# flynn-nrg/izpi

Measured on AMD Instinct MI355X. Metric: Msamples/sec (pixels x spp) at 1024x1024/512spp, higher is better.
Workload: dtype f64

## Files before the change

### include/izpi_gpu.h

```cpp
#ifndef IZPI_GPU_H
#define IZPI_GPU_H
#include <stddef.h>
#include <stdint.h>
#include "izpi_types.h"

#ifdef __cplusplus
extern "C" {
#endif

typedef struct izpi_ctx izpi_ctx;

typedef struct izpi_scene_desc {
  uint32_t abi_version;
  uint32_t num_nodes;
  uint32_t num_prims;
  uint32_t num_tris, num_spheres, num_lights, num_materials, num_textures;
  uint32_t num_spd;
  uint32_t flags;
  uint64_t num_texels;
  const izpi_bvh4_node* nodes;
  const uint32_t* prim_ref;
  const double* tri_v0;
  const double* tri_v1;
  const double* tri_v2;
// ... 29 lines not shown
  IZPI_SAMPLER_WIREFRAME = 3,
  IZPI_SAMPLER_ALBEDO = 4,
  IZPI_SAMPLER_SPECTRAL = 5
};
enum {
  IZPI_OUT_CANVAS = 0,
  IZPI_OUT_PACKED = 1
};

typedef struct izpi_render_tuning {
  uint32_t slots;
  uint32_t chunk_units;
  uint32_t rec_dense;
  uint32_t pool_div;
  uint32_t trace_chunk;
  uint32_t refill_min;
  uint32_t prim_weight;
  uint32_t flags;
  uint64_t tail_paths;
  uint32_t peer_timeout_ms;
  uint32_t pad_tuning;
} izpi_render_tuning;
enum {
  IZPI_TUNE_NO_DIST = 1,
  IZPI_TUNE_GENERAL_TRACE = 2,
  IZPI_TUNE_NO_LEAF_SHORTCUT = 4,
  IZPI_TUNE_SCALAR_SLAB = 8,
  IZPI_TUNE_NO_TAIL = 16,
  IZPI_TUNE_PASS_LOG = 32,
  IZPI_TUNE_NO_LDS_BVH = 64,
  IZPI_TUNE_NO_RAY_LDS = 128,
  IZPI_TUNE_NO_PRIM_LDS = 256,
  IZPI_TUNE_NO_PLACE_PICK = 512,
  IZPI_TUNE_NO_QNODES = 1024
};

typedef struct izpi_render_req {
  uint32_t width, height;
  uint32_t spp;
  uint32_t max_depth;
  uint32_t sampler;
  uint32_t out_layout;
  uint32_t num_tiles;
  uint32_t num_bg_spd;
  const uint32_t* tiles;
  const double* bg_spd_wavelengths;
  const double* bg_spd_values;
  double background[3];
  uint64_t seed;
  uint32_t post;
  uint32_t abi_version;
  double exposure;
  const izpi_render_tuning* tuning;
  uint32_t accumulation;
  uint32_t pad_req;
  double ink[3];
} izpi_render_req;

enum { IZPI_ACC_RECURSIVE = 0, IZPI_ACC_FORWARD = 1 };

enum { IZPI_POST_NONE = 0, IZPI_POST_SPECTRAL = 1,
       IZPI_POST_GAMMA_CLAMP = 2 };

enum { IZPI_FILTER_GAMMA = 1,
       IZPI_FILTER_CLAMP = 2   };
#define IZPI_MAX_FILTERS 8

// ... 85 lines not shown
```

### izpi_amd/_native.py

```python
import ctypes as C
from pathlib import Path

ROOT = Path(__file__).resolve().parents[1]
LIB_PATH = ROOT / "izpi_amd" / "_lib" / "libizpi_gpu.so"

c_double_p = C.POINTER(C.c_double)
c_uint32_p = C.POINTER(C.c_uint32)
c_float_p = C.POINTER(C.c_float)

COMM_ID_BYTES = 128
IZPI_OK, IZPI_ERR_INVALID, IZPI_ERR_HIP, IZPI_ERR_NO_SCENE, IZPI_ERR_UNSUPPORTED, IZPI_ERR_DEVICE, IZPI_ERR_PEER = range(7)
IZPI_ABI_VERSION = 4
ACC_RECURSIVE, ACC_FORWARD = 0, 1
SCENE_QUANTIZED_BVH = 1
PRIM_TRIANGLE, PRIM_SPHERE = 0, 1
TEX_CONSTANT, TEX_IMAGE, TEX_SPECTRAL_GAUSSIAN, TEX_SPECTRAL_TABULATED, TEX_SPECTRAL_IMAGE = 1, 3, 5, 7, 9
MAT_DIELECTRIC, MAT_DIFFUSE_LIGHT, MAT_ISOTROPIC, MAT_LAMBERT, MAT_METAL, MAT_PBR = 1, 2, 3, 4, 5, 6
MATF_BEER_LAMBERT = 1
SAMPLER_NORMAL, SAMPLER_COLOUR, SAMPLER_WIREFRAME, SAMPLER_ALBEDO, SAMPLER_SPECTRAL = 1, 2, 3, 4, 5
OUT_CANVAS, OUT_PACKED = 0, 1
POST_NONE, POST_SPECTRAL, POST_GAMMA_CLAMP = 0, 1, 2
FILTER_GAMMA, FILTER_CLAMP = 1, 2
MAX_FILTERS = 8
HOST_SKIP_BVH = 1
# ... 31 lines not shown
                ("vertical", C.c_double * 3), ("u", C.c_double * 3), ("v", C.c_double * 3),
                ("lens_radius", C.c_double), ("time0", C.c_double), ("time1", C.c_double), ("exposure", C.c_double)]


class SceneDesc(C.Structure):
    _fields_ = [("abi_version", C.c_uint32), ("num_nodes", C.c_uint32), ("num_prims", C.c_uint32),
                ("num_tris", C.c_uint32), ("num_spheres", C.c_uint32), ("num_lights", C.c_uint32),
                ("num_materials", C.c_uint32), ("num_textures", C.c_uint32), ("num_spd", C.c_uint32),
                ("flags", C.c_uint32), ("num_texels", C.c_uint64),
                ("nodes", C.POINTER(BVH4Node)), ("prim_ref", c_uint32_p),
                ("tri_v0", c_double_p), ("tri_v1", c_double_p), ("tri_v2", c_double_p),
                ("tri_e1", c_double_p), ("tri_e2", c_double_p), ("tri_normal", c_double_p),
                ("tri_tangent", c_double_p), ("tri_bitangent", c_double_p), ("tri_uv", c_double_p),
                ("tri_area", c_double_p), ("tri_mat", c_uint32_p),
                ("sph_center0", c_double_p), ("sph_center1", c_double_p), ("sph_time", c_double_p),
                ("sph_radius", c_double_p), ("sph_mat", c_uint32_p),
                ("light_ref", c_uint32_p), ("materials", C.POINTER(Material)), ("textures", C.POINTER(Texture)),
                ("texels", c_double_p), ("spd_wavelengths", c_double_p), ("spd_values", c_double_p),
                ("camera", Camera)]


class RenderTuning(C.Structure):
    _fields_ = [("slots", C.c_uint32), ("chunk_units", C.c_uint32), ("rec_dense", C.c_uint32),
                ("pool_div", C.c_uint32), ("trace_chunk", C.c_uint32), ("refill_min", C.c_uint32),
                ("prim_weight", C.c_uint32), ("flags", C.c_uint32), ("tail_paths", C.c_uint64),
                ("peer_timeout_ms", C.c_uint32), ("pad_tuning", C.c_uint32)]


TUNE_NO_DIST, TUNE_GENERAL_TRACE, TUNE_NO_LEAF_SHORTCUT, TUNE_SCALAR_SLAB, TUNE_NO_TAIL, TUNE_PASS_LOG = 1, 2, 4, 8, 16, 32
TUNE_NO_LDS_BVH = 64
TUNE_NO_RAY_LDS = 128
TUNE_NO_PRIM_LDS = 256
TUNE_NO_QNODES = 1024


def tuning(**kw):
    t = RenderTuning()
    for k, v in kw.items():
        if k == "flags" and not isinstance(v, int):
            v = sum(v)
        setattr(t, k, v)
    return t


class RenderReq(C.Structure):
    _fields_ = [("width", C.c_uint32), ("height", C.c_uint32), ("spp", C.c_uint32), ("max_depth", C.c_uint32),
                ("sampler", C.c_uint32), ("out_layout", C.c_uint32), ("num_tiles", C.c_uint32),
                ("num_bg_spd", C.c_uint32), ("tiles", c_uint32_p), ("bg_spd_wavelengths", c_double_p),
                ("bg_spd_values", c_double_p), ("background", C.c_double * 3), ("seed", C.c_uint64),
                ("post", C.c_uint32), ("abi_version", C.c_uint32), ("exposure", C.c_double),
                ("tuning", C.POINTER(RenderTuning)), ("accumulation", C.c_uint32), ("pad_req", C.c_uint32),
                ("ink", C.c_double * 3)]


class RenderStats(C.Structure):
    _fields_ = [("rays", C.c_uint64), ("node_visits", C.c_uint64), ("tri_tests", C.c_uint64),
                ("sph_tests", C.c_uint64), ("light_tri_tests", C.c_uint64), ("light_sph_tests", C.c_uint64),
                ("samples", C.c_uint64), ("kernel_ms", C.c_double), ("shade_ms", C.c_double),
                ("total_ms", C.c_double), ("launches", C.c_uint32), ("pad", C.c_uint32),
                ("node_steps", C.c_uint64), ("prim_steps", C.c_uint64), ("leaf_shortcuts", C.c_uint64),
                ("tail_ms", C.c_double), ("tail_node_visits", C.c_uint64), ("tail_tri_tests", C.c_uint64),
                ("tail_sph_tests", C.c_uint64), ("parks", C.c_uint64), ("workspace_bytes", C.c_uint64),
                ("scene_bytes", C.c_uint64), ("slots", C.c_uint32), ("rec_dense", C.c_uint32),
                ("pool_blocks", C.c_uint32), ("chunk_spp", C.c_uint32), ("alloc_ms", C.c_double)]

    def as_dict(self):
# ... 200 lines not shown
```

### izpi_amd/csrc/izpi_gpu.hip

```cpp
#include "izpi_kern.h"

__global__ void __launch_bounds__(256) k_spectral_post(const double* in, double* out, uint32_t W, uint32_t H,
                                                       double exposure) {
  __shared__ double ys[18][18];
  const int tx = threadIdx.x & 15, ty = threadIdx.x >> 4;
  const int x0 = blockIdx.x * 16, y0 = blockIdx.y * 16;
  for (int i = threadIdx.x; i < 18 * 18; i += 256) {
    const int hx = x0 + (i % 18) - 1, hy = y0 + (i / 18) - 1;
    ys[i / 18][i % 18] = (hx >= 0 && hx < (int)W && hy >= 0 && hy < (int)H) ? in[((size_t)hy * W + hx) * 4 + 1] : 0.0;
  }
  __syncthreads();
  const int x = x0 + tx, y = y0 + ty;
  if (x >= (int)W || y >= (int)H) return;
  const size_t pi = ((size_t)y * W + x) * 4;
  const double2 xy = *reinterpret_cast<const double2*>(in + pi), za = *reinterpret_cast<const double2*>(in + pi + 2);
  double X = xy.x, Y = xy.y, Z = za.x;
  const double cur = ys[ty + 1][tx + 1];
  if (cur > 0) {
    double nb[8];
    int nn = 0;
    for (int dy = -1; dy <= 1; dy++)
      for (int dx = -1; dx <= 1; dx++) {
        if (dx == 0 && dy == 0) continue;
        const int nx = x + dx, ny = y + dy;
// ... 634 lines not shown
    return IZPI_OK;
  }
  if (tu.flags & IZPI_TUNE_PASS_LOG) HIP_TRY(hipEventRecord(ctx->evb[0], ctx->stream));
  WaveBuf bufs[2];
  carve_state(ctx->d_state, slots, need_time, rec_pool != 0, need_cold, need_uv, thr_planes, bufs);
  hipStream_t st = ctx->stream;
  HIP_TRY(hipMemcpyAsync(ctx->d_tiles, tiles.data(), tiles.size() * sizeof(uint32_t), hipMemcpyHostToDevice, st));
  if (nbg) {
    HIP_TRY(hipMemcpyAsync(ctx->d_bg, req->bg_spd_wavelengths, nbg * sizeof(double), hipMemcpyHostToDevice, st));
    HIP_TRY(hipMemcpyAsync(ctx->d_bg + nbg, req->bg_spd_values, nbg * sizeof(double), hipMemcpyHostToDevice, st));
  }
  HIP_TRY(hipMemsetAsync(ctx->d_running, 0, (size_t)num_pixels * 3 * sizeof(double), st));
  HIP_TRY(hipMemsetAsync(ctx->d_counters, 0, CNT_N * sizeof(unsigned long long), st));
  HIP_TRY(hipMemsetAsync(ctx->d_cpart, 0, (size_t)cpart_rows * CNT_N * sizeof(unsigned long long), st));
  HIP_TRY(hipMemsetAsync(ctx->d_misc, 0, 8 * MISC_STRIDE * sizeof(uint32_t), st));

  ShadeParams sp{};
  sp.width = req->width; sp.height = req->height; sp.max_depth = req->max_depth;
  sp.tile_w = tw; sp.tile_h = th; sp.num_bg_spd = (uint32_t)nbg; sp.slots = slots;
  sp.bg_sorted = nbg >= 2;
  for (size_t i = 1; i < nbg; i++)
    if (!(req->bg_spd_wavelengths[i - 1] <= req->bg_spd_wavelengths[i])) sp.bg_sorted = 0;
  sp.tiles = ctx->d_tiles; sp.bg_wl = ctx->d_bg; sp.bg_val = ctx->d_bg + nbg;
  sp.background[0] = req->background[0]; sp.background[1] = req->background[1]; sp.background[2] = req->background[2];
  sp.rec_dense = rec_dense; sp.rec_pool = rec_pool;
  sp.pool_shift = 0;
  while (pool_blocks && (POOL_SHARDS << sp.pool_shift) < pool_blocks) sp.pool_shift++;
  sp.seed = req->seed; sp.out = ctx->d_samples; sp.recs = fwd ? nullptr : ctx->d_recs; sp.mat_const = sc.mat_const; sp.head = misc(ctx, 0);
  sp.num_mc = ctx->num_materials; sp.num_tex = ctx->num_textures; sp.num_spd = ctx->num_spd;
  sp.staged = ctx->num_materials <= MC_LDS && ctx->num_materials <= MAT_LDS && sc.num_lights <= LT_LDS &&
              ctx->num_textures <= TEX_LDS && ctx->num_spd <= SPD_LDS && nbg <= BG_LDS;
  sp.prims_staged = sc.num_prims <= PR_LDS && !(tuning_of(req).flags & IZPI_TUNE_NO_PRIM_LDS);
  if (sp.staged && (req->sampler == IZPI_SAMPLER_SPECTRAL || ctx->num_spd)) sp.staged = 2;
  sc.lds_bytes = sp.prims_staged ? lds_off::END : sp.staged == 2 ? lds_off::SPECTRAL_END : sp.staged ? lds_off::COLOUR_END : 0;
  sp.pool = rec_pool ? ctx->d_pool : nullptr; sp.pool_ring = rec_pool ? ctx->d_ring : nullptr;
  sp.pool_ctr = rec_pool ? ctx->d_pool_ctr : nullptr;
  sp.counters = ctx->d_counters; sp.cpart = ctx->d_cpart; sp.error = misc(ctx, 1);
  sp.finq = ctx->d_finq;
  WaveParams wp{};
  wp.in = bufs[0]; wp.out = bufs[1]; wp.trace_next = misc(ctx, 2); wp.slots = slots;
  wp.read_kind = !ctx->sc.no_pathlen ? 1u : 0u;
  wp.hit_uv = need_uv ? 1u : 0u;
  wp.pool_ctr = sp.pool_ctr;
  wp.cpart = ctx->d_cpart;
  AccumParams ap{};
  ap.num_pixels = num_pixels; ap.spp = req->spp; ap.width = req->width; ap.height = req->height;
  ap.tile_w = tw; ap.tile_h = th; ap.sampler = req->sampler; ap.out_layout = req->out_layout;
  ap.tiles = ctx->d_tiles; ap.samples = ctx->d_samples; ap.running = ctx->d_running; ap.out = out_dev;

  float trace_ms = 0, shade_ms = 0, tail_ms = 0;
  uint32_t launches = 0;
  const double t_launch = host_ms();
  HIP_TRY(hipEventRecord(ctx->ev0, st));
  if (tu.flags & IZPI_TUNE_PASS_LOG) {
    HIP_TRY(hipEventSynchronize(ctx->ev0));
    float prep = 0;
    HIP_TRY(hipEventElapsedTime(&prep, ctx->evb[0], ctx->ev0));
    fprintf(stderr, "IZPI_T ev0_synced %.3f prep_gpu_ms %.3f body_start %.3f\n", diag_clock_ms(), prep,
            diag_clock_ms() - host_ms());
  }
#define IZPI_RUN(S, F) run_sampler<S, F>(ctx, req, sc, tr, sp, wp, ap, num_pixels, chunk, pool_blocks, compact, &trace_ms, &shade_ms, \
                                        &tail_ms, &launches)
  if (req->sampler == IZPI_SAMPLER_COLOUR) rc = fwd ? IZPI_RUN(IZPI_SAMPLER_COLOUR, true) : IZPI_RUN(IZPI_SAMPLER_COLOUR, false);
  else rc = fwd ? IZPI_RUN(IZPI_SAMPLER_SPECTRAL, true) : IZPI_RUN(IZPI_SAMPLER_SPECTRAL, false);
#undef IZPI_RUN
  if (rc) return rc;
// ... 1139 lines not shown
```

### izpi_amd/csrc/izpi_kern.h

```cpp
#pragma once
#include <hip/hip_runtime.h>
#include <stdio.h>
#include <stdlib.h>
#include <string.h>
#include <algorithm>
#include <cmath>
#include <string>
#include <vector>

#include <rccl/rccl.h>

#include <atomic>
#include <chrono>
#include <thread>

#include "../../include/izpi_host.h"
#include "../../include/izpi_gpu_debug.h"
#include "izpi_dev.h"
#include "izpi_req.h"
#include "cie_tables.h"

using namespace izd;

#define HIP_TRY(expr)                                                                  \
// ... 55 lines not shown
#pragma unroll
    for (uint32_t i = 0; i < sizeof(T) / 8; i++) d[i] = q[i];
    return r;
  } else {
    return *(const __attribute__((address_space(3))) T*)p;
  }
}

template <bool L, class T>
IZPI_DEV T tld(const T* p) {
  if constexpr (L) return lds_ld(p);
  else return *p;
}
constexpr uint32_t MAT_LDS = 64, TEX_LDS = 64, SPD_LDS = 384, BG_LDS = 128, MT_LDS = 64, LT_LDS = 64, PR_LDS = 64;
namespace lds_off {
constexpr uint32_t al(uint64_t b) { return (uint32_t)((b + 31) & ~31ull); }
constexpr uint32_t MC = 0;
constexpr uint32_t MT = MC + al(MT_LDS * sizeof(double4));
constexpr uint32_t LT = MT + al(MT_LDS * sizeof(MatTex));
constexpr uint32_t LT2 = LT + al(LT_LDS * 16 * sizeof(double));
constexpr uint32_t MAT = LT2 + al(LT_LDS * 6 * sizeof(double));
constexpr uint32_t TEX = MAT + al(MAT_LDS * sizeof(izpi_material));
constexpr uint32_t COLOUR_END = TEX + al(TEX_LDS * sizeof(izpi_texture));
constexpr uint32_t SPD = COLOUR_END;
constexpr uint32_t SPDV = SPD + al(SPD_LDS * sizeof(double));
constexpr uint32_t CIE = SPDV + al(SPD_LDS * sizeof(double));
constexpr uint32_t BG = CIE + al(5 * IZPI_CIE_N * sizeof(double));
constexpr uint32_t BGV = BG + al(BG_LDS * sizeof(double));
constexpr uint32_t SPECTRAL_END = BGV + al(BG_LDS * sizeof(double));
constexpr uint32_t GS = SPECTRAL_END;
constexpr uint32_t TT = GS + al(PR_LDS * sizeof(GShade));
constexpr uint32_t GP = TT + al(PR_LDS * sizeof(GTriTex));
constexpr uint32_t END = GP + al(PR_LDS * sizeof(GPrim));
}
IZPI_DEV char* lds_arena() {
  extern __shared__ __attribute__((aligned(16))) char izpi_lds_arena[];
  return izpi_lds_arena;
}
IZPI_DEV izpi_material* mat_lds() { return (izpi_material*)(lds_arena() + lds_off::MAT); }
IZPI_DEV izpi_texture* tex_lds() { return (izpi_texture*)(lds_arena() + lds_off::TEX); }
IZPI_DEV double* spd_lds() { return (double*)(lds_arena() + lds_off::SPD); }
IZPI_DEV double* spdv_lds() { return (double*)(lds_arena() + lds_off::SPDV); }
IZPI_DEV double* cie_lds() { return (double*)(lds_arena() + lds_off::CIE); }
IZPI_DEV double* bg_lds() { return (double*)(lds_arena() + lds_off::BG); }
IZPI_DEV double* bgv_lds() { return (double*)(lds_arena() + lds_off::BGV); }
IZPI_DEV izpi_material mat_rec(const DevScene& sc, bool st, uint32_t m) {
  if (st) return lds_ld(mat_lds() + m);
  return sc.materials[m];
}
IZPI_DEV izpi_texture tex_rec(const DevScene& sc, bool st, int32_t id) {
  if (st) return lds_ld(tex_lds() + id);
  return sc.textures[id];
}

IZPI_DEV V3 image_rgb(const double* texels, uint64_t off, uint32_t w, uint32_t h, uint32_t fmt, double u, double v) {
  int64_t i = go_int(u * (double)w);
  int64_t j = go_int((1 - v) * ((double)h - 0.001));
  if (i < 0) i = 0;
  if (j < 0) j = 0;
  if (i > (int64_t)w - 1) i = (int64_t)w - 1;
  if (j > (int64_t)h - 1) j = (int64_t)h - 1;
  uint64_t k = (uint64_t)j * w + (uint64_t)i;
  if (fmt == TEXF_GRAY) {
    const double g = texels[off + k];
    return mk(g, g, g);
  }
// ... 1150 lines not shown
```

### izpi_amd/csrc/shade.h

```cpp
#pragma once
#include "izpi_kern.h"

template <int SAMPLER, bool FWD>
__global__ void __launch_bounds__(256) k_start(const DevScene sc, const ShadeParams sp_in, const WaveParams wp) {
  ShadeParams sp = sp_in;
  sp.staged = 0;
  sp.prims_staged = 0;
  const uint32_t j = blockIdx.x * 256 + threadIdx.x;
  bool want = j < sp.slots;
  bool push = false;
  bool first = true;
  PathSt P;
  RayRec R;
  P.rslot = j;
  for (;;) {
    uint32_t unit;
    if (first) {
      unit = (want && j < sp.total_units) ? j : 0xFFFFFFFFu;
      first = false;
    } else {
      unit = grab_unit(sp, want);
    }
    if (__ballot(want) == 0) break;
    if (want) {
// ... 68 lines not shown
  if (threadIdx.x == 0) {
    const uint32_t ne = np + nu;
    if (nu && u0 + nu >= sp.total_units) exhausted = true;
    s_pbase[b] = pb;
    s_ubase[b] = u0;
    s_granted[b] = u0 >= sp.total_units ? 0u : min(nu, sp.total_units - u0);
    s_nput[b] = np;
    s_nent[b] = ne;
    SCLK_VMWAIT();
    SCLK_ADD(SCLK_RATOM, rb1);
  }
  __syncthreads();
  SCLK_ADD(SCLK_RB2, rb1);
  uint32_t ur = (uint32_t)__popcll(mu & lt), pr = (uint32_t)__popcll(mp & lt);
  for (uint32_t i = 0; i < w; i++) { ur += s_u[b][i]; pr += s_p[b][i]; }
  if constexpr (QSEP) {
    q_rank = (uint32_t)__popcll(mq & lt);
    q_total = 0;
#pragma unroll
    for (uint32_t k = 0; k < SHADE_WAVES; k++) {
      q_rank += k < w ? s_q[b][k] : 0u;
      q_total += s_q[b][k];
    }
  } else {
    q_rank = ur;
    q_total = 0;
#pragma unroll
    for (uint32_t k = 0; k < SHADE_WAVES; k++) q_total += s_u[b][k];
  }
  const bool has_entry = unit_want && s_nput[b] + ur < s_nent[b];
  const bool granted = unit_want && ur < s_granted[b];
  unit = granted ? s_ubase[b] + ur : 0xFFFFFFFFu;
  pos = put ? s_pbase[b] + pr : (has_entry ? s_pbase[b] + s_nput[b] + ur : 0xFFFFFFFFu);
}

template <int SAMPLER, bool FWD>
IZPI_DEV void refill_one(const DevScene& sc, const ShadeParams& sp, const WaveBuf& out, uint32_t unit, uint32_t pos,
                         PathSt& P) {
  RayRec R;
  for (;;) {
    if (start_path<SAMPLER, FWD>(sc, sp, unit, P, R)) {
      store_entry<SAMPLER, FWD>(out, pos, P, R);
      return;
    }
    unit = atomicAdd(sp.head, 1u);
    if (unit >= sp.total_units) {
      dead_entry(out, pos);
      return;
    }
  }
}




template <int SAMPLER, int MATSET, bool DEFER, bool FWD>
IZPI_DEV void shade_item(const DevScene& sc, const ShadeParams& sp, const WaveBuf& in, uint32_t i, uint32_t kind,
                         const EntryIn& E, PathSt& P, RayRec& R, bool& push, bool& done, uint32_t& fblk, uint32_t& c_lt,
                         uint32_t& c_ls, bool& queued) {
  const bool COLOUR = SAMPLER == IZPI_SAMPLER_COLOUR;
  const bool st = sp.staged != 0;
  SCLK_T(sc0);
  SCLK_VMWAIT();
  SCLK_ADD(SCLK_ENTRY, sc0);
  for (int k = 0; k < 3; k++) { R.o[k] = E.ray.o[k]; R.d[k] = E.ray.d[k]; }
  R.kind = kind;
// ... 263 lines not shown
    const unsigned long long idx = atomicAdd(c, 1ull);
    if (idx < __atomic_load_n(c + 2, __ATOMIC_RELAXED)) return sp.pool_ring[((size_t)ring << sp.pool_shift) + (idx & size_mask)] + 1u;
  }
  return 0u;
}

template <int SAMPLER>
IZPI_DEV void fin_queue(unsigned long long* q, uint32_t j, const PathSt& P, const RayRec& R) {
  const bool colour = SAMPLER == IZPI_SAMPLER_COLOUR;
  q[j] = P.unit | (unsigned long long)P.rslot << 32;
  q[FINQ_CAP + j] = P.blk | (unsigned long long)(P.depth | P.zf << 16) << 32;
  q[2 * FINQ_CAP + j] = (unsigned long long)__double_as_longlong(R.o[0]);
  q[3 * FINQ_CAP + j] = (unsigned long long)__double_as_longlong(colour ? R.o[1] : P.lambda);
  q[4 * FINQ_CAP + j] = (unsigned long long)__double_as_longlong(colour ? R.o[2] : P.lpdf);
}
template <int SAMPLER, int MATSET>
IZPI_DEV void fin_flush(const ShadeParams& sp, const unsigned long long* q, uint32_t n) {
  const bool colour = SAMPLER == IZPI_SAMPLER_COLOUR;
  for (uint32_t j = threadIdx.x; j < n; j += SHADE_THREADS) {
    PathSt P;
    const unsigned long long w0 = q[j], w1 = q[FINQ_CAP + j];
    P.unit = (uint32_t)w0; P.rslot = (uint32_t)(w0 >> 32);
    P.blk = (uint32_t)w1; P.depth = (uint32_t)(w1 >> 32) & 0xFFFFu; P.zf = (uint32_t)(w1 >> 48);
    const double a = __longlong_as_double((long long)q[2 * FINQ_CAP + j]);
    const double b = __longlong_as_double((long long)q[3 * FINQ_CAP + j]);
    const double c = __longlong_as_double((long long)q[4 * FINQ_CAP + j]);
    P.lambda = colour ? 0.0 : b; P.lpdf = colour ? 0.0 : c;
    finish<SAMPLER, MATSET>(sp, P, colour ? mk(a, b, c) : mk(a, 0.0, 0.0));
    if (sp.rec_pool && P.blk) pool_free_one(sp, P.blk);
  }
}

constexpr int SHADE_WPE = 3;
template <int SAMPLER, int MATSET, bool FWD>
__global__ void __launch_bounds__(SHADE_THREADS) __attribute__((amdgpu_waves_per_eu(SHADE_WPE)))
k_shade(const DevScene sc, const ShadeParams sp, const WaveParams wp) {
  constexpr bool DREF = FWD;
  shade_stage(sc, sp);
  uint32_t parity = 0;
  const uint32_t n = *wp.in_count;
  const uint32_t cam_b = FWD && wp.cam ? wp.cam[0] : 0u, cam_u = FWD && wp.cam ? wp.cam[1] : 0u,
                 cam_m = FWD && wp.cam ? wp.cam[2] : 0u;
  if (blockIdx.x == 0 && threadIdx.x == 0) *wp.trace_next = 0;
  bool exhausted = false;
  uint32_t c_lt = 0, c_ls = 0, c_park = 0;
  const uint32_t stride = gridDim.x * SHADE_THREADS;
  constexpr bool DEFER = !FWD && (SAMPLER == IZPI_SAMPLER_SPECTRAL || ms_spec(MATSET));
  constexpr bool COLOUR_DEFER = DEFER && SAMPLER == IZPI_SAMPLER_COLOUR;
  unsigned long long* fq = sp.finq + (size_t)blockIdx.x * FINQ_WORDS * FINQ_CAP;
  uint32_t fq_n = 0;
#ifdef IZPI_SHADE_CLOCKS
  uint64_t k_item = 0, k_ref = 0, k_push = 0;
  sclk_zero();
#endif
  for (uint32_t base = blockIdx.x * SHADE_THREADS; base < n; base += stride) {
    const uint32_t i = base + threadIdx.x;
    const bool valid = i < n;
    bool push = false;
    bool done = false;
    bool parked = false;
    uint32_t fblk = 0;
#ifdef IZPI_SHADE_CLOCKS
    uint64_t t0 = __builtin_readcyclecounter();
#endif
    PathSt P;
    RayRec R;
    P.rslot = 0; P.blk = 0; P.depth = 0; P.zf = 0;
    uint32_t kind = RAY_DEAD;
    EntryIn E;
    if (valid) {
      kind = sld(wp.in.kind + i) & ~(uint32_t)RAY_PARKED;
      if (FWD && i - cam_b < cam_m) camera_path<SAMPLER>(sp, cam_u + (i - cam_b), P);
      else load_path<SAMPLER, FWD>(wp.in, i, P);
      load_entry(wp.in, i, E);
    }
    const bool live = valid && !(kind & RAY_DEAD);
    if (sp.rec_pool) {
      const bool need = live && P.depth >= sp.rec_dense && P.blk == 0;
      const uint32_t b = pool_alloc(sp, need);
      P.blk = need ? b : P.blk;
      parked = need && b == 0;
      c_park += parked ? 1u : 0u;
    }
    bool queued = false;
    if (live && !parked) shade_item<SAMPLER, MATSET, DEFER, FWD>(sc, sp, wp.in, i, kind, E, P, R, push, done, fblk, c_lt, c_ls, queued);
    if (SAMPLER == IZPI_SAMPLER_SPECTRAL) queued = DEFER && done;
    if ((COLOUR_DEFER ? !queued : !DEFER) && sp.rec_pool && fblk) pool_free_one(sp, fblk);
#ifdef IZPI_SHADE_CLOCKS
    uint64_t t1 = __builtin_readcyclecounter();
    k_item += t1 - t0;
    t0 = t1;
#endif
    uint32_t unit, pos, frank, ftotal;
    block_reserve2<COLOUR_DEFER>(sp, wp.out_count, push || parked, done && !DREF, unit, pos, parity, exhausted, queued, frank,
                                 ftotal);
    if (queued) fin_queue<SAMPLER>(fq, fq_n + frank, P, R);
    fq_n += ftotal;
    if (push) store_entry<SAMPLER, FWD>(wp.out, pos, P, R);
    if (parked) copy_entry(wp.in, i, wp.out, pos);
#ifdef IZPI_SHADE_CLOCKS
    t1 = __builtin_readcyclecounter();
    k_push += t1 - t0;
    t0 = t1;
#endif
    if constexpr (!DREF) {
      if (unit != 0xFFFFFFFFu) refill_one<SAMPLER, FWD>(sc, sp, wp.out, unit, pos, P);
      else if (done && pos != 0xFFFFFFFFu) dead_entry(wp.out, pos);
    }
#ifdef IZPI_SHADE_CLOCKS
    t1 = __builtin_readcyclecounter();
    k_ref += t1 - t0;
#endif
    if (DEFER && fq_n >= FINQ_FLUSH) {
      __syncthreads();
      fin_flush<SAMPLER, MATSET>(sp, fq, fq_n);
      fq_n = 0;
    }
  }
  if (DEFER && fq_n) {
    __syncthreads();
    fin_flush<SAMPLER, MATSET>(sp, fq, fq_n);
  }
  const uint32_t lane = threadIdx.x & 63;
#ifdef IZPI_SHADE_CLOCKS
  if (lane == 0) {
    atomicAdd(sp.counters + CNT_SCLK_ITEM, (unsigned long long)k_item);
    atomicAdd(sp.counters + CNT_SCLK_REFILL, (unsigned long long)k_ref);
    atomicAdd(sp.counters + CNT_SCLK_PUSH, (unsigned long long)k_push);
  }
  sclk_flush(sp.counters);
#endif
  if (c_park && wp.out_park) *wp.out_park = 1u;
  unsigned long long vals[3] = {c_lt, c_ls, c_park};
  const int idx[3] = {CNT_LTRI, CNT_LSPH, CNT_PARK};
  for (int k = 0; k < 3; k++) {
    unsigned long long s = vals[k];
    for (int off = 32; off > 0; off >>= 1) s += __shfl_down(s, off);
    if (lane == 0) count_add(sp.cpart, sp.counters, idx[k], s);
  }
}

constexpr uint32_t REFILL_ALIGN = 64;
static __global__ void k_plan_first(uint32_t* out_count, uint32_t* plan, uint32_t fill) {
  plan[0] = 0; plan[1] = 0; plan[2] = fill; plan[3] = 0;
  *out_count = fill;
}
static __global__ void k_refill_plan(const ShadeParams sp, uint32_t* out_count, uint32_t* plan) {
  const uint32_t nc = *out_count, h = *sp.head;
  const uint32_t base = min((nc + (REFILL_ALIGN - 1)) / REFILL_ALIGN * REFILL_ALIGN, sp.slots);
  const uint32_t room = sp.slots - base;
  const uint32_t m = h < sp.total_units ? min(room, sp.total_units - h) : 0u;
  plan[0] = m ? base : nc; plan[1] = h; plan[2] = m; plan[3] = nc;
  *out_count = m ? base + m : nc;
  *sp.head = h + m;
// ... 133 lines not shown
  if (ap.sampler == IZPI_SAMPLER_COLOUR) {
    r0 = c0 / (double)ap.spp; r1 = c1 / (double)ap.spp; r2 = c2 / (double)ap.spp;
  } else {
    const double inv = 1.0 / (double)ap.spp;
    r0 = c0 * inv; r1 = c1 * inv; r2 = c2 * inv;
  }
  const uint32_t tile_px = ap.tile_w * ap.tile_h;
  if (ap.out_layout == IZPI_OUT_PACKED) {
    double* o = ap.out + (size_t)p * 4;
    o[0] = r0; o[1] = r1; o[2] = r2; o[3] = 1.0;
    return;
  }
  const uint32_t tile = p / tile_px, in_tile = p % tile_px;
  const uint32_t x = ap.tiles[4 * tile] + in_tile % ap.tile_w;
  const uint32_t y = ap.tiles[4 * tile + 1] + in_tile / ap.tile_w;
  const uint32_t row = ap.height - y;
  if (row < ap.height) {
    double* o = ap.out + ((size_t)row * ap.width + x) * 4;
    o[0] = r0; o[1] = r1; o[2] = r2; o[3] = 1.0;
  }
}


template <int SAMPLER, int MATSET, bool FWD>
int run_chunks(izpi_ctx* ctx, const izpi_render_req* req, const DevScene& sc, const Tracer& tr, ShadeParams& sp,
               WaveParams& wp, AccumParams& ap, uint32_t num_pixels, uint32_t chunk, uint32_t pool_blocks,
               float* trace_ms, float* shade_ms, float* tail_ms, uint32_t* launches) {
  hipStream_t st = ctx->stream;
  const izpi_render_tuning& tu = tuning_of(req);
  int shade_res = 0;
  const size_t dyn = sc.lds_bytes;
  int rc = resident_blocks(ctx, k_shade<SAMPLER, MATSET, FWD>, &shade_res, (int)SHADE_THREADS, dyn);
  if (rc) return rc;
  const bool tail_deep = ctx->stack_needed > 32;
  int tail_res = 0;
  if ((rc = tail_deep ? resident_blocks(ctx, k_tail<SAMPLER, MATSET, 64, FWD>, &tail_res, 256, dyn)
                      : resident_blocks(ctx, k_tail<SAMPLER, MATSET, 32, FWD>, &tail_res, 256, dyn))) return rc;
  if ((uint32_t)std::max({tr.blocks * 4, shade_res * (int)SHADE_WAVES, tail_res * 4}) > ctx->num_cus * CPART_BLOCKS_PER_CU * 4 ||
      (uint32_t)shade_res > ctx->num_cus * CPART_BLOCKS_PER_CU) {
    ctx->err = "grid larger than the counter rows or the unwinding queues";
    return IZPI_ERR_INVALID;
  }
  if (tail_deep && (size_t)tail_res * 256 * (64 - TAIL_LDS_STACK) * sizeof(int32_t) > ctx->spill_cap) {
    ctx->err = "k_tail's stack spill does not fit k_trace2's spill area";
    return IZPI_ERR_INVALID;
  }
  int refill_res = 0;
  if constexpr (FWD)
    if ((rc = resident_blocks(ctx, k_refill<SAMPLER>, &refill_res, 256, 0))) return rc;
  uint64_t tail_max = (uint64_t)tail_res * 256;
  if (tu.tail_paths) tail_max = tu.tail_paths;
  if (tu.flags & IZPI_TUNE_NO_TAIL) tail_max = 0;
  if (sp.rec_pool) tail_max = std::min<uint64_t>(tail_max, pool_blocks);
  const WaveBuf q[2] = {wp.in, wp.out};
  uint32_t* qn[2] = {misc(ctx, 3), misc(ctx, 4)};
  if (sp.rec_pool)
    hipLaunchKernelGGL(k_pool_init, dim3((pool_blocks + 255) / 256), dim3(256), 0, st, sp.pool_ring, pool_blocks,
                       pool_blocks / POOL_SHARDS, sp.pool_ctr);
  HIP_TRY(hipGetLastError());
  for (uint32_t s0 = 0; s0 < req->spp; s0 += chunk) {
    const uint32_t cs = std::min(chunk, req->spp - s0);
    sp.chunk_spp = cs; sp.s0 = s0; sp.total_units = num_pixels * cs;
    const uint32_t fill = std::min<uint32_t>(sp.slots, sp.total_units);
    HIP_TRY(hipMemsetD32Async(misc(ctx, 0), (int)fill, 1, st));
    HIP_TRY(hipMemsetAsync(misc(ctx, 2), 0, 3 * MISC_STRIDE * sizeof(uint32_t), st));
    HIP_TRY(hipMemsetAsync(misc(ctx, 6), 0, 2 * MISC_STRIDE * sizeof(uint32_t), st));
    wp.out = q[0]; wp.out_count = qn[0];
    if constexpr (FWD) {
      hipLaunchKernelGGL(k_plan_first, dim3(1), dim3(1), 0, st, wp.out_count, misc(ctx, 5), fill);
      hipLaunchKernelGGL(k_refill<SAMPLER>, dim3(refill_res), dim3(256), 0, st, sc, sp, wp, (const uint32_t*)misc(ctx, 5));
    } else {
      hipLaunchKernelGGL((k_start<SAMPLER, FWD>), dim3((fill + 255) / 256), dim3(256), 0, st, sc, sp, wp);
    }
    HIP_TRY(hipGetLastError());
    HIP_TRY(hipMemcpyAsync(ctx->h_count, qn[0], sizeof(uint32_t), hipMemcpyDeviceToHost, st));
    HIP_TRY(hipStreamSynchronize(st));
    if (tu.flags & IZPI_TUNE_PASS_LOG) fprintf(stderr, "IZPI_T start_synced %.3f\n", diag_clock_ms());
    uint32_t n = ctx->h_count[0];
    int cur = 0;
    const bool pass_log = (tu.flags & IZPI_TUNE_PASS_LOG) != 0;
    int B = pass_log ? 1 : IZPI_PASS_BATCH;
    while (n > 0) {
      for (int b = 0; b < B; b++) {
        wp.in = q[cur]; wp.in_count = qn[cur];
        wp.out = q[1 - cur]; wp.out_count = qn[1 - cur];
        wp.in_park = misc(ctx, 6 + cur); wp.out_park = misc(ctx, 6 + (1 - cur));
        wp.cam = FWD ? misc(ctx, 5) : nullptr;
        HIP_TRY(hipEventRecord(ctx->evb[3 * b], st));
        launch_trace(ctx, sc, tr, wp, st, ctx->d_spill);
        HIP_TRY(hipGetLastError());
        HIP_TRY(hipEventRecord(ctx->evb[3 * b + 1], st));
        hipLaunchKernelGGL((k_shade<SAMPLER, MATSET, FWD>), dim3(shade_res), dim3(SHADE_THREADS), dyn, st, sc, sp, wp);
        HIP_TRY(hipGetLastError());
        if constexpr (FWD) {
          hipLaunchKernelGGL(k_refill_plan, dim3(1), dim3(1), 0, st, sp, wp.out_count, misc(ctx, 5));
          hipLaunchKernelGGL(k_refill<SAMPLER>, dim3(refill_res), dim3(256), 0, st, sc, sp, wp, (const uint32_t*)misc(ctx, 5));
          HIP_TRY(hipGetLastError());
        }
        HIP_TRY(hipEventRecord(ctx->evb[3 * b + 2], st));
        cur = 1 - cur;
      }
      HIP_TRY(hipMemcpyAsync(ctx->h_count, ctx->d_misc, 8 * MISC_STRIDE * sizeof(uint32_t), hipMemcpyDeviceToHost, st));
      HIP_TRY(hipStreamSynchronize(st));
      for (int b = 0; b < B; b++) {
        float t_ms = 0, s_ms = 0;
        HIP_TRY(hipEventElapsedTime(&t_ms, ctx->evb[3 * b], ctx->evb[3 * b + 1]));
        HIP_TRY(hipEventElapsedTime(&s_ms, ctx->evb[3 * b + 1], ctx->evb[3 * b + 2]));
        *trace_ms += t_ms;
        *shade_ms += s_ms;
        if (pass_log) fprintf(stderr, "IZPI_PASS %u trace %.3f shade %.3f\n", *launches, t_ms, s_ms);
        (*launches)++;
      }
      const uint32_t head = ctx->h_count[0];
      n = ctx->h_count[(3 + cur) * MISC_STRIDE];
      {
        const uint64_t started = std::min<uint64_t>(head, sp.total_units);
        ctx->prog_done.store((uint64_t)s0 * num_pixels + (started > n ? started - n : 0), std::memory_order_relaxed);
      }
      if (pass_log) fprintf(stderr, "IZPI_BATCH queue %u head %u\n", n, head);
      if (head >= sp.total_units) B = 1;
      if (n > 0 && n <= tail_max && head >= sp.total_units) {
        wp.in = q[cur]; wp.in_count = qn[cur];
        HIP_TRY(hipEventRecord(ctx->ev2, st));
        if (sp.rec_pool) hipLaunchKernelGGL(k_pool_publish, dim3(1), dim3(256), 0, st, sp.pool_ctr);
        if (tail_deep) hipLaunchKernelGGL((k_tail<SAMPLER, MATSET, 64, FWD>), dim3(tail_res), dim3(256), dyn, st, sc, sp, wp, ctx->d_spill);
// ... 11 lines not shown
    ap.raw_spectral = FWD && SAMPLER == IZPI_SAMPLER_SPECTRAL ? 1u : 0u;
    ap.last = (s0 + cs >= req->spp) ? 1u : 0u;
    ctx->prog_done.store((uint64_t)(s0 + cs) * num_pixels, std::memory_order_relaxed);
    hipLaunchKernelGGL(k_accumulate, dim3((num_pixels + 255) / 256), dim3(256), 0, st, ap);
    HIP_TRY(hipGetLastError());
  }
  return IZPI_OK;
}


template <int SAMPLER, bool FWD>
int run_sampler(izpi_ctx* ctx, const izpi_render_req* req, const DevScene& sc, const Tracer& tr, ShadeParams& sp,
                WaveParams& wp, AccumParams& ap, uint32_t num_pixels, uint32_t chunk, uint32_t pool_blocks, bool compact,
                float* trace_ms, float* shade_ms, float* tail_ms, uint32_t* launches) {
#define IZPI_RUN(M) run_chunks<SAMPLER, M, FWD>(ctx, req, sc, tr, sp, wp, ap, num_pixels, chunk, pool_blocks, trace_ms, shade_ms, tail_ms, launches)
  const uint32_t ms = ctx->matset;
  const int set = ms == 0 ? MATSET_BASIC : (ms & ~(uint32_t)MATSET_SURF) == 0 ? MATSET_SURF : MATSET_FULL;
  if constexpr (SAMPLER == IZPI_SAMPLER_COLOUR && !FWD)
    if (compact) return IZPI_RUN(MATSET_CONST);
  return set == MATSET_BASIC ? IZPI_RUN(MATSET_BASIC) : set == MATSET_SURF ? IZPI_RUN(MATSET_SURF) : IZPI_RUN(MATSET_FULL);
#undef IZPI_RUN
}

template <int SAMPLER, bool FWD>
int prepare_sampler(izpi_ctx* ctx, bool compact) {
  const uint32_t ms = ctx->matset;
  const int set = ms == 0 ? MATSET_BASIC : (ms & ~(uint32_t)MATSET_SURF) == 0 ? MATSET_SURF : MATSET_FULL;
  int blocks = 0, rc = IZPI_OK;
  auto query = [&](auto shade, auto tail32, auto tail64) {
    if ((rc = resident_blocks(ctx, shade, &blocks, (int)SHADE_THREADS))) return;
    if ((rc = resident_blocks(ctx, tail32, &blocks))) return;
    rc = resident_blocks(ctx, tail64, &blocks);
  };
#define IZPI_Q(M) query(k_shade<SAMPLER, M, FWD>, k_tail<SAMPLER, M, 32, FWD>, k_tail<SAMPLER, M, 64, FWD>)
  bool done = false;
  if constexpr (SAMPLER == IZPI_SAMPLER_COLOUR && !FWD)
    if (compact) { IZPI_Q(MATSET_CONST); done = true; }
  if (done) {
  } else if (set == MATSET_BASIC) IZPI_Q(MATSET_BASIC);
  else if (set == MATSET_SURF) IZPI_Q(MATSET_SURF);
  else IZPI_Q(MATSET_FULL);
#undef IZPI_Q
  if (rc) return rc;
  if ((rc = resident_blocks(ctx, k_start<SAMPLER, FWD>, &blocks))) return rc;
  if constexpr (FWD)
    if ((rc = resident_blocks(ctx, k_refill<SAMPLER>, &blocks))) return rc;
  return resident_blocks(ctx, k_accumulate, &blocks);
}
```

Baseline: 2356.

## Stage shade output entries in LDS and flush them coalesced every other iteration

Adds a staged variant of the forward colour shade kernel. On alternating iterations each block compacts its pushed path entries into LDS. On the next iteration it reserves one combined output range with a single atomic and writes the staged entries as contiguous, coalesced stores alongside the current iteration's entries. This halves the per-block atomic reservations and improves store coalescing, at the cost of extra LDS, extra barriers and a final flush. For eligible scenes it also disables primitive LDS staging so the arena fits. The variant is used only when occupancy stays unchanged, and a tuning flag can turn it off.

```diff
diff --git a/include/izpi_gpu.h b/include/izpi_gpu.h
--- a/include/izpi_gpu.h
+++ b/include/izpi_gpu.h
@@ -85,7 +85,8 @@
   IZPI_TUNE_NO_RAY_LDS = 128,
   IZPI_TUNE_NO_PRIM_LDS = 256,
   IZPI_TUNE_NO_PLACE_PICK = 512,
-  IZPI_TUNE_NO_QNODES = 1024
+  IZPI_TUNE_NO_QNODES = 1024,
+  IZPI_TUNE_NO_SHADE_STAGE = 2048
 };
 
 typedef struct izpi_render_req {
diff --git a/izpi_amd/_native.py b/izpi_amd/_native.py
--- a/izpi_amd/_native.py
+++ b/izpi_amd/_native.py
@@ -87,6 +87,7 @@
 TUNE_NO_RAY_LDS = 128
 TUNE_NO_PRIM_LDS = 256
 TUNE_NO_QNODES = 1024
+TUNE_NO_SHADE_STAGE = 2048
 
 
 def tuning(**kw):
diff --git a/izpi_amd/csrc/izpi_gpu.hip b/izpi_amd/csrc/izpi_gpu.hip
--- a/izpi_amd/csrc/izpi_gpu.hip
+++ b/izpi_amd/csrc/izpi_gpu.hip
@@ -690,6 +690,9 @@
               ctx->num_textures <= TEX_LDS && ctx->num_spd <= SPD_LDS && nbg <= BG_LDS;
   sp.prims_staged = sc.num_prims <= PR_LDS && !(tuning_of(req).flags & IZPI_TUNE_NO_PRIM_LDS);
   if (sp.staged && (req->sampler == IZPI_SAMPLER_SPECTRAL || ctx->num_spd)) sp.staged = 2;
+  if (fwd && req->sampler == IZPI_SAMPLER_COLOUR && ctx->matset == 0 && sp.staged == 1 && !rec_pool && !need_time && !need_cold &&
+      !(tuning_of(req).flags & IZPI_TUNE_NO_SHADE_STAGE))
+    sp.prims_staged = 0;
   sc.lds_bytes = sp.prims_staged ? lds_off::END : sp.staged == 2 ? lds_off::SPECTRAL_END : sp.staged ? lds_off::COLOUR_END : 0;
   sp.pool = rec_pool ? ctx->d_pool : nullptr; sp.pool_ring = rec_pool ? ctx->d_ring : nullptr;
   sp.pool_ctr = rec_pool ? ctx->d_pool_ctr : nullptr;
diff --git a/izpi_amd/csrc/izpi_kern.h b/izpi_amd/csrc/izpi_kern.h
--- a/izpi_amd/csrc/izpi_kern.h
+++ b/izpi_amd/csrc/izpi_kern.h
@@ -111,6 +111,12 @@
 constexpr uint32_t TT = GS + al(PR_LDS * sizeof(GShade));
 constexpr uint32_t GP = TT + al(PR_LDS * sizeof(GTriTex));
 constexpr uint32_t END = GP + al(PR_LDS * sizeof(GPrim));
+constexpr uint32_t STG_RAY = COLOUR_END;
+constexpr uint32_t STG_THR = STG_RAY + 3 * SHADE_THREADS * 16;
+constexpr uint32_t STG_PATH = STG_THR + 3 * SHADE_THREADS * 8;
+constexpr uint32_t STG_KIND = STG_PATH + SHADE_THREADS * 16;
+constexpr uint32_t STG_END = STG_KIND + SHADE_THREADS * 4;
+constexpr uint32_t STG_BYTES = STG_END - COLOUR_END;
 }
 IZPI_DEV char* lds_arena() {
   extern __shared__ __attribute__((aligned(16))) char izpi_lds_arena[];
diff --git a/izpi_amd/csrc/shade.h b/izpi_amd/csrc/shade.h
--- a/izpi_amd/csrc/shade.h
+++ b/izpi_amd/csrc/shade.h
@@ -124,6 +124,81 @@
   const bool granted = unit_want && ur < s_granted[b];
   unit = granted ? s_ubase[b] + ur : 0xFFFFFFFFu;
   pos = put ? s_pbase[b] + pr : (has_entry ? s_pbase[b] + s_nput[b] + ur : 0xFFFFFFFFu);
+}
+
+typedef double stg_d2 __attribute__((ext_vector_type(2)));
+typedef uint32_t stg_u4 __attribute__((ext_vector_type(4)));
+#define IZPI_LDS3 __attribute__((address_space(3)))
+IZPI_DEV IZPI_LDS3 stg_d2* stg_ray() { return (IZPI_LDS3 stg_d2*)(lds_arena() + lds_off::STG_RAY); }
+IZPI_DEV IZPI_LDS3 double* stg_thr() { return (IZPI_LDS3 double*)(lds_arena() + lds_off::STG_THR); }
+IZPI_DEV IZPI_LDS3 stg_u4* stg_path() { return (IZPI_LDS3 stg_u4*)(lds_arena() + lds_off::STG_PATH); }
+IZPI_DEV IZPI_LDS3 uint32_t* stg_kind() { return (IZPI_LDS3 uint32_t*)(lds_arena() + lds_off::STG_KIND); }
+IZPI_DEV uint32_t stage_put(bool put, const PathSt& P, const RayRec& R) {
+  __shared__ uint32_t s_n[SHADE_WAVES];
+  const uint32_t w = threadIdx.x >> 6, lane = threadIdx.x & 63;
+  const uint64_t mp = __ballot(put);
+  if (lane == 0) s_n[w] = (uint32_t)__popcll(mp);
+  SCLK_T(rb0);
+  __syncthreads();
+  SCLK_ADD(SCLK_RB1, rb0);
+  uint32_t r = (uint32_t)__popcll(mp & ((1ull << lane) - 1)), n = 0;
+#pragma unroll
+  for (uint32_t k = 0; k < SHADE_WAVES; k++) {
+    r += k < w ? s_n[k] : 0u;
+    n += s_n[k];
+  }
+  if (put) {
+    stg_ray()[r] = stg_d2{R.o[0], R.o[1]};
+    stg_ray()[SHADE_THREADS + r] = stg_d2{R.o[2], R.d[0]};
+    stg_ray()[2 * SHADE_THREADS + r] = stg_d2{R.d[1], R.d[2]};
+    stg_thr()[r] = P.thr[0];
+    stg_thr()[SHADE_THREADS + r] = P.thr[1];
+    stg_thr()[2 * SHADE_THREADS + r] = P.thr[2];
+    stg_path()[r] = stg_u4{P.rng, P.depth | P.zf << 16, P.unit, P.rslot};
+    stg_kind()[r] = R.kind;
+  }
+  return n;
+}
+IZPI_DEV void block_reserve_fwd(uint32_t* out_count, bool put, uint32_t staged, uint32_t& base, uint32_t& rank) {
+  __shared__ uint32_t s_p[SHADE_WAVES], s_base;
+  const uint32_t w = threadIdx.x >> 6, lane = threadIdx.x & 63;
+  const uint64_t mp = __ballot(put);
+  if (lane == 0) s_p[w] = (uint32_t)__popcll(mp);
+  SCLK_T(rb0);
+  __syncthreads();
+  SCLK_ADD(SCLK_RB1, rb0);
+  SCLK_T(rb1);
+  if (threadIdx.x == 0) {
+    uint32_t ne = staged;
+#pragma unroll
+    for (uint32_t k = 0; k < SHADE_WAVES; k++) ne += s_p[k];
+    s_base = ne ? atomicAdd(out_count, ne) : 0u;
+    SCLK_VMWAIT();
+    SCLK_ADD(SCLK_RATOM, rb1);
+  }
+  __syncthreads();
+  SCLK_ADD(SCLK_RB2, rb1);
+  rank = (uint32_t)__popcll(mp & ((1ull << lane) - 1));
+  for (uint32_t k = 0; k < w; k++) rank += s_p[k];
+  base = s_base;
+}
+IZPI_DEV void stage_flush(const WaveBuf& out, uint32_t base, uint32_t n) {
+  const uint32_t t = threadIdx.x;
+  if (t >= n) return;
+  const uint32_t pos = base + t;
+  const stg_d2 r0 = stg_ray()[t], r1 = stg_ray()[SHADE_THREADS + t], r2 = stg_ray()[2 * SHADE_THREADS + t];
+  const double t0 = stg_thr()[t], t1 = stg_thr()[SHADE_THREADS + t], t2 = stg_thr()[2 * SHADE_THREADS + t];
+  const stg_u4 ph = stg_path()[t];
+  const uint32_t kind = stg_kind()[t];
+  sst(out.thr + pos, t0);
+  sst(out.thr + out.tplane + pos, t1);
+  sst(out.thr + 2 * (size_t)out.tplane + pos, t2);
+  double2* r = reinterpret_cast<double2*>(out.ray + pos);
+  sst(r, make_double2(r0.x, r0.y));
+  sst(r + 1, make_double2(r1.x, r1.y));
+  sst(r + 2, make_double2(r2.x, r2.y));
+  sst(out.kind + pos, kind);
+  sst(out.path + pos, PathHot{ph.x, ph.y, ph.z, ph.w});
 }
 
 template <int SAMPLER, bool FWD>
@@ -453,12 +528,17 @@
 }
 
 constexpr int SHADE_WPE = 3;
-template <int SAMPLER, int MATSET, bool FWD>
+constexpr bool shade_can_stage(int sampler, int matset, bool fwd) {
+  return fwd && sampler == IZPI_SAMPLER_COLOUR && matset != MATSET_FULL;
+}
+template <int SAMPLER, int MATSET, bool FWD, bool STAGE = false>
 __global__ void __launch_bounds__(SHADE_THREADS) __attribute__((amdgpu_waves_per_eu(SHADE_WPE)))
 k_shade(const DevScene sc, const ShadeParams sp, const WaveParams wp) {
+  static_assert(!STAGE || shade_can_stage(SAMPLER, MATSET, FWD), "no staged form of this instance");
   constexpr bool DREF = FWD;
   shade_stage(sc, sp);
   uint32_t parity = 0;
+  uint32_t st_phase = 0, st_n = 0;
   const uint32_t n = *wp.in_count;
   const uint32_t cam_b = FWD && wp.cam ? wp.cam[0] : 0u, cam_u = FWD && wp.cam ? wp.cam[1] : 0u,
                  cam_m = FWD && wp.cam ? wp.cam[2] : 0u;
@@ -512,13 +592,25 @@
     k_item += t1 - t0;
     t0 = t1;
 #endif
-    uint32_t unit, pos, frank, ftotal;
-    block_reserve2<COLOUR_DEFER>(sp, wp.out_count, push || parked, done && !DREF, unit, pos, parity, exhausted, queued, frank,
-                                 ftotal);
-    if (queued) fin_queue<SAMPLER>(fq, fq_n + frank, P, R);
-    fq_n += ftotal;
-    if (push) store_entry<SAMPLER, FWD>(wp.out, pos, P, R);
-    if (parked) copy_entry(wp.in, i, wp.out, pos);
+    uint32_t unit = 0xFFFFFFFFu, pos = 0xFFFFFFFFu, frank = 0, ftotal = 0;
+    if constexpr (STAGE) {
+      if (st_phase == 0) {
+        st_n = stage_put(push, P, R);
+      } else {
+        uint32_t rbase, rank;
+        block_reserve_fwd(wp.out_count, push, st_n, rbase, rank);
+        if (push) store_entry<SAMPLER, FWD>(wp.out, rbase + st_n + rank, P, R);
+        stage_flush(wp.out, rbase, st_n);
+      }
+      st_phase ^= 1u;
+    } else {
+      block_reserve2<COLOUR_DEFER>(sp, wp.out_count, push || parked, done && !DREF, unit, pos, parity, exhausted, queued, frank,
+                                   ftotal);
+      if (queued) fin_queue<SAMPLER>(fq, fq_n + frank, P, R);
+      fq_n += ftotal;
+      if (push) store_entry<SAMPLER, FWD>(wp.out, pos, P, R);
+      if (parked) copy_entry(wp.in, i, wp.out, pos);
+    }
 #ifdef IZPI_SHADE_CLOCKS
     t1 = __builtin_readcyclecounter();
     k_push += t1 - t0;
@@ -541,6 +633,13 @@
   if (DEFER && fq_n) {
     __syncthreads();
     fin_flush<SAMPLER, MATSET>(sp, fq, fq_n);
+  }
+  if constexpr (STAGE) {
+    if (st_phase) {
+      uint32_t rbase, rank;
+      block_reserve_fwd(wp.out_count, false, st_n, rbase, rank);
+      stage_flush(wp.out, rbase, st_n);
+    }
   }
   const uint32_t lane = threadIdx.x & 63;
 #ifdef IZPI_SHADE_CLOCKS
@@ -740,6 +839,20 @@
   const size_t dyn = sc.lds_bytes;
   int rc = resident_blocks(ctx, k_shade<SAMPLER, MATSET, FWD>, &shade_res, (int)SHADE_THREADS, dyn);
   if (rc) return rc;
+  bool stage = false;
+  const char* form = "plain (no staged instance)";
+  if constexpr (shade_can_stage(SAMPLER, MATSET, FWD)) {
+    if (tu.flags & IZPI_TUNE_NO_SHADE_STAGE) form = "plain (IZPI_TUNE_NO_SHADE_STAGE)";
+    else if (sp.rec_pool || sc.lds_bytes != lds_off::COLOUR_END) form = "plain (LDS arena)";
+    else if (wp.out.time || wp.out.blk || wp.out.cold || !wp.out.thr) form = "plain (entry arrays)";
+    else {
+      int stage_res = 0;
+      if ((rc = resident_blocks(ctx, k_shade<SAMPLER, MATSET, FWD, true>, &stage_res, (int)SHADE_THREADS, dyn + lds_off::STG_BYTES))) return rc;
+      stage = stage_res == shade_res;
+      form = stage ? "staged" : "plain (occupancy)";
+    }
+  }
+  if (tu.flags & IZPI_TUNE_PASS_LOG) fprintf(stderr, "IZPI_SHADE_FORM %s\n", form);
   const bool tail_deep = ctx->stack_needed > 32;
   int tail_res = 0;
   if ((rc = tail_deep ? resident_blocks(ctx, k_tail<SAMPLER, MATSET, 64, FWD>, &tail_res, 256, dyn)
@@ -798,7 +911,13 @@
         launch_trace(ctx, sc, tr, wp, st, ctx->d_spill);
         HIP_TRY(hipGetLastError());
         HIP_TRY(hipEventRecord(ctx->evb[3 * b + 1], st));
-        hipLaunchKernelGGL((k_shade<SAMPLER, MATSET, FWD>), dim3(shade_res), dim3(SHADE_THREADS), dyn, st, sc, sp, wp);
+        bool launched = false;
+        if constexpr (shade_can_stage(SAMPLER, MATSET, FWD))
+          if (stage) {
+            hipLaunchKernelGGL((k_shade<SAMPLER, MATSET, FWD, true>), dim3(shade_res), dim3(SHADE_THREADS), dyn + lds_off::STG_BYTES, st, sc, sp, wp);
+            launched = true;
+          }
+        if (!launched) hipLaunchKernelGGL((k_shade<SAMPLER, MATSET, FWD>), dim3(shade_res), dim3(SHADE_THREADS), dyn, st, sc, sp, wp);
         HIP_TRY(hipGetLastError());
         if constexpr (FWD) {
           hipLaunchKernelGGL(k_refill_plan, dim3(1), dim3(1), 0, st, sp, wp.out_count, misc(ctx, 5));
@@ -876,7 +995,15 @@
     if ((rc = resident_blocks(ctx, tail32, &blocks))) return;
     rc = resident_blocks(ctx, tail64, &blocks);
   };
-#define IZPI_Q(M) query(k_shade<SAMPLER, M, FWD>, k_tail<SAMPLER, M, 32, FWD>, k_tail<SAMPLER, M, 64, FWD>)
+  auto query_staged = [&](auto shade) {
+    if (!rc) rc = resident_blocks(ctx, shade, &blocks, (int)SHADE_THREADS);
+  };
+  (void)query_staged;
+#define IZPI_Q(M)                                                                                             \
+  do {                                                                                                        \
+    query(k_shade<SAMPLER, M, FWD>, k_tail<SAMPLER, M, 32, FWD>, k_tail<SAMPLER, M, 64, FWD>);                \
+    if constexpr (shade_can_stage(SAMPLER, M, FWD)) query_staged(k_shade<SAMPLER, M, FWD, true>);             \
+  } while (0)
   bool done = false;
   if constexpr (SAMPLER == IZPI_SAMPLER_COLOUR && !FWD)
     if (compact) { IZPI_Q(MATSET_CONST); done = true; }
```

New measurement: 2427 (median of 6 runs). +3.0%, better.
